# KristinnVikarJ/nbody-simulation

Measured on AMD Instinct MI355X. Metric: pair-interactions/sec + ms/step at N=1M direct O(N^2) (force + integration step), higher is better.
Workload: dtype f32; 1 GPU; direct O(N^2) f32, N=1048576 bodies, seeded 2-D Plummer sphere, masses 1, dt=0.1, clamp=0.001 (BASELINE.json configs[2]); n_bodies=1048576, targets_per_gpu=1048576, n_ranks=1, entry=one process per GPU (sharding.py over nbody_direct_{prep,run}_dev), exchange=none, arith=AUTO (FAST kernel; EXACT on hazardous positions)

## Files before the change

### nbody-simulation_amd/csrc/direct_mutual.hip

```cpp
#include <hip/hip_runtime.h>
#include <stdint.h>

#include "direct_kernels.h"
#include "mutual_schedule.h"

namespace nbody {

namespace {

typedef float v2f __attribute__((ext_vector_type(2)));

constexpr int kWaves = 8;

constexpr int kSlice = kMutualSlice;
constexpr int kSliceCouples = kSlice / 2;
constexpr int kChunks = kSliceCouples / 64;
constexpr float kMarker = 1e30f;

__device__ __forceinline__ bool gate_open(const DirectArgs& a) { return a.run_state < 0 || a.flags[kFlagState] == a.run_state; }

__device__ __forceinline__ float4 couple_or_marker(const float4* c, int64_t k, int64_t n_couples) {
  return k < n_couples ? c[k] : make_float4(kMarker, kMarker, kMarker, kMarker);
}

#define NB_PX(K, H, D) "v_pk_add_f32 v[" D "], v[184:185], %[tx" #K "] op_sel:[0," #H "] op_sel_hi:[1," #H "] neg_lo:[0,1] neg_hi:[0,1]\n\t"
#define NB_PY(K, H, D) "v_pk_add_f32 v[" D "], v[186:187], %[ty" #K "] op_sel:[0," #H "] op_sel_hi:[1," #H "] neg_lo:[0,1] neg_hi:[0,1]\n\t"
#define NB_SQ(DX, DY, Q) "v_pk_mul_f32 v[" Q "], v[" DX "], v[" DX "]\n\tv_pk_fma_f32 v[" Q "], v[" DY "], v[" DY "], v[" Q "]\n\t"
#define NB_AD(XL, XH, YL, YH, SL, SH) "v_add_f32_e64 v" SL ", |v" XL "|, |v" YL "|\n\tv_add_f32_e64 v" SH ", |v" XH "|, |v" YH "|\n\t"
#define NB_DN(S, Q) "v_pk_fma_f32 v[" S "], v[" S "], v[" Q "], %[b]\n\t"
#define NB_RC(SL, SH) "v_rcp_f32_e32 v" SL ", v" SL "\n\tv_rcp_f32_e32 v" SH ", v" SH "\n\t"
#define NB_AC(T, DX, DY, S)                                                                                                          \
  "v_pk_fma_f32 %[ax" #T "], v[" DX "], v[" S "], %[ax" #T "]\n\t"                                                                    \
  "v_pk_fma_f32 v[188:189], v[" DX "], v[" S "], v[188:189] neg_lo:[1,0,0] neg_hi:[1,0,0]\n\t"                                                  \
  "v_pk_fma_f32 %[ay" #T "], v[" DY "], v[" S "], %[ay" #T "]\n\t"                                                                    \
  "v_pk_fma_f32 v[190:191], v[" DY "], v[" S "], v[190:191] neg_lo:[1,0,0] neg_hi:[1,0,0]\n\t"
#define NB_HALF(K0, K1, K2, K3, T0, T1, T2, T3, T4, T5, T6, T7)                                                                    \
  NB_PX(K0, 0, "192:193") NB_PX(K0, 1, "200:201") NB_PX(K1, 0, "208:209") NB_PX(K1, 1, "216:217")                                   \
  NB_PX(K2, 0, "224:225") NB_PX(K2, 1, "232:233") NB_PX(K3, 0, "240:241") NB_PX(K3, 1, "248:249")                                   \
  NB_PY(K0, 0, "194:195") NB_PY(K0, 1, "202:203") NB_PY(K1, 0, "210:211") NB_PY(K1, 1, "218:219")                                   \
  NB_PY(K2, 0, "226:227") NB_PY(K2, 1, "234:235") NB_PY(K3, 0, "242:243") NB_PY(K3, 1, "250:251")                                   \
  NB_SQ("192:193", "194:195", "196:197") NB_SQ("200:201", "202:203", "204:205") NB_SQ("208:209", "210:211", "212:213")             \
  NB_SQ("216:217", "218:219", "220:221") NB_SQ("224:225", "226:227", "228:229") NB_SQ("232:233", "234:235", "236:237")             \
  NB_SQ("240:241", "242:243", "244:245") NB_SQ("248:249", "250:251", "252:253")                                                    \
  "s_setprio 0\n\t"                                                                                                                \
  NB_AD("192", "193", "194", "195", "198", "199") NB_AD("200", "201", "202", "203", "206", "207")                                  \
  NB_AD("208", "209", "210", "211", "214", "215") NB_AD("216", "217", "218", "219", "222", "223")                                  \
  NB_AD("224", "225", "226", "227", "230", "231") NB_AD("232", "233", "234", "235", "238", "239")                                  \
  NB_AD("240", "241", "242", "243", "246", "247") NB_AD("248", "249", "250", "251", "254", "255")                                  \
  "s_setprio 1\n\t"                                                                                                                \
  NB_DN("198:199", "196:197") NB_DN("206:207", "204:205") NB_DN("214:215", "212:213") NB_DN("222:223", "220:221")                 \
  NB_DN("230:231", "228:229") NB_DN("238:239", "236:237") NB_DN("246:247", "244:245") NB_DN("254:255", "252:253")                 \
  NB_RC("198", "199")                                                                                                              \
  NB_RC("206", "207") NB_AC(T0, "192:193", "194:195", "198:199")                                                                   \
  NB_RC("214", "215") NB_AC(T1, "200:201", "202:203", "206:207")                                                                   \
  NB_RC("222", "223") NB_AC(T2, "208:209", "210:211", "214:215")                                                                   \
  NB_RC("230", "231") NB_AC(T3, "216:217", "218:219", "222:223")                                                                   \
  NB_RC("238", "239") NB_AC(T4, "224:225", "226:227", "230:231")                                                                   \
  NB_RC("246", "247") NB_AC(T5, "232:233", "234:235", "238:239")                                                                   \
  NB_RC("254", "255") NB_AC(T6, "240:241", "242:243", "246:247")                                                                   \
  NB_AC(T7, "248:249", "250:251", "254:255")
#define NB_ROT(R) "v_mov_b32_dpp " R ", " R " wave_ror:1 row_mask:0xf bank_mask:0xf\n\t"

__device__ __forceinline__ void mutual_steps(const v2f* tx, const v2f* ty, v2f* ax, v2f* ay, float4& rc, float4& sacc, int steps,
                                             unsigned long long bias2) {
  asm volatile("v_mov_b32 v184, %[r0]\n\tv_mov_b32 v185, %[r1]\n\tv_mov_b32 v186, %[r2]\n\tv_mov_b32 v187, %[r3]\n\t"
               "v_mov_b32 v188, %[o0]\n\tv_mov_b32 v189, %[o1]\n\tv_mov_b32 v190, %[o2]\n\tv_mov_b32 v191, %[o3]\n\t"
               "s_mov_b32 s88, %[n]\n"
               ".Lnb_mutual_%=:\n\t"
               NB_HALF(0, 1, 2, 3, 0, 1, 2, 3, 4, 5, 6, 7) NB_HALF(4, 5, 6, 7, 8, 9, 10, 11, 12, 13, 14, 15)
               NB_ROT("v184") NB_ROT("v185") NB_ROT("v186") NB_ROT("v187") NB_ROT("v188") NB_ROT("v189") NB_ROT("v190") NB_ROT("v191")
               "s_sub_u32 s88, s88, 1\n\t"
               "s_cmp_lg_u32 s88, 0\n\t"
               "s_cbranch_scc1 .Lnb_mutual_%=\n\t"
               "v_mov_b32 %[o0], v188\n\tv_mov_b32 %[o1], v189\n\tv_mov_b32 %[o2], v190\n\tv_mov_b32 %[o3], v191\n\t"
               "v_mov_b32 %[r0], v184\n\tv_mov_b32 %[r1], v185\n\tv_mov_b32 %[r2], v186\n\tv_mov_b32 %[r3], v187\n\t"
               : [ax0] "+v"(ax[0]), [ax1] "+v"(ax[1]), [ax2] "+v"(ax[2]), [ax3] "+v"(ax[3]), [ax4] "+v"(ax[4]), [ax5] "+v"(ax[5]),
                 [ax6] "+v"(ax[6]), [ax7] "+v"(ax[7]), [ax8] "+v"(ax[8]), [ax9] "+v"(ax[9]), [ax10] "+v"(ax[10]), [ax11] "+v"(ax[11]),
                 [ax12] "+v"(ax[12]), [ax13] "+v"(ax[13]), [ax14] "+v"(ax[14]), [ax15] "+v"(ax[15]),
                 [ay0] "+v"(ay[0]), [ay1] "+v"(ay[1]), [ay2] "+v"(ay[2]), [ay3] "+v"(ay[3]), [ay4] "+v"(ay[4]), [ay5] "+v"(ay[5]),
                 [ay6] "+v"(ay[6]), [ay7] "+v"(ay[7]), [ay8] "+v"(ay[8]), [ay9] "+v"(ay[9]), [ay10] "+v"(ay[10]), [ay11] "+v"(ay[11]),
                 [ay12] "+v"(ay[12]), [ay13] "+v"(ay[13]), [ay14] "+v"(ay[14]), [ay15] "+v"(ay[15]),
                 [o0] "+v"(sacc.x), [o1] "+v"(sacc.y), [o2] "+v"(sacc.z), [o3] "+v"(sacc.w),
                 [r0] "+v"(rc.x), [r1] "+v"(rc.y), [r2] "+v"(rc.z), [r3] "+v"(rc.w)
               : [tx0] "v"(tx[0]), [tx1] "v"(tx[1]), [tx2] "v"(tx[2]), [tx3] "v"(tx[3]), [tx4] "v"(tx[4]), [tx5] "v"(tx[5]),
                 [tx6] "v"(tx[6]), [tx7] "v"(tx[7]), [ty0] "v"(ty[0]), [ty1] "v"(ty[1]), [ty2] "v"(ty[2]), [ty3] "v"(ty[3]),
                 [ty4] "v"(ty[4]), [ty5] "v"(ty[5]), [ty6] "v"(ty[6]), [ty7] "v"(ty[7]), [b] "s"(bias2), [n] "s"(steps)
               : "v184", "v185", "v186", "v187", "v188", "v189", "v190", "v191",
                 "v192", "v193", "v194", "v195", "v196", "v197", "v198", "v199", "v200", "v201", "v202", "v203", "v204", "v205",
                 "v206", "v207", "v208", "v209", "v210", "v211", "v212", "v213", "v214", "v215", "v216", "v217", "v218", "v219",
                 "v220", "v221", "v222", "v223", "v224", "v225", "v226", "v227", "v228", "v229", "v230", "v231", "v232", "v233",
                 "v234", "v235", "v236", "v237", "v238", "v239", "v240", "v241", "v242", "v243", "v244", "v245", "v246", "v247",
                 "v248", "v249", "v250", "v251", "v252", "v253", "v254", "v255", "s88", "scc");
}
#undef NB_PX
#undef NB_PY
#undef NB_SQ
#undef NB_AD
#undef NB_DN
#undef NB_RC
#undef NB_AC
#undef NB_HALF
#undef NB_ROT

__device__ __forceinline__ void load_targets(const float4* couples, int64_t n_couples, int s, int w, int lane, v2f* tx, v2f* ty) {
  const int64_t tc0 = (int64_t)s * kSliceCouples + 512 * w + 8 * lane;
#pragma unroll
  for (int k = 0; k < 8; ++k) {
    const float4 c = couple_or_marker(couples, tc0 + k, n_couples);
    tx[k] = v2f{c.x, c.y};
    ty[k] = v2f{c.z, c.w};
  }
}

__device__ __forceinline__ void zero_acc(v2f* ax, v2f* ay) {
#pragma unroll
  for (int t = 0; t < 16; ++t) ax[t] = ay[t] = v2f{0.f, 0.f};
}

__device__ __forceinline__ void add_chunk(const v2f* ax, const v2f* ay, float* tot_x, float* tot_y) {
#pragma unroll
  for (int t = 0; t < 16; ++t) {
    tot_x[t] += ax[t].x + ax[t].y;
    tot_y[t] += ay[t].x + ay[t].y;
  }
}

constexpr unsigned long long kBias2 = 0x1280000012800000ull;

__device__ __forceinline__ void off_item(const float4* couples, int64_t n_couples, int s, int b, int w, int lane, float4 (*red)[kWaves][64],
                                         float2* tpart, float2* spart_f2) {
  v2f tx[8], ty[8];
  load_targets(couples, n_couples, s, w, lane, tx, ty);
  float tot_x[16], tot_y[16];
#pragma unroll
  for (int t = 0; t < 16; ++t) tot_x[t] = tot_y[t] = 0.f;
  float* spart = reinterpret_cast<float*>(spart_f2);
  for (int c = 0; c < kChunks; ++c) {
    float4 rc = couple_or_marker(couples, (int64_t)b * kSliceCouples + 64 * c + lane, n_couples);
    v2f ax[16], ay[16];
    zero_acc(ax, ay);
    float4 sacc = make_float4(0.f, 0.f, 0.f, 0.f);
    mutual_steps(tx, ty, ax, ay, rc, sacc, 64, kBias2);
    add_chunk(ax, ay, tot_x, tot_y);
    red[c & 1][w][lane] = sacc;
    __syncthreads();
    if (threadIdx.x < 256) {
      const int q = threadIdx.x >> 2, comp = threadIdx.x & 3;
      float r = 0.f;
#pragma unroll
      for (int v = 0; v < kWaves; ++v) r += reinterpret_cast<const float*>(&red[c & 1][v][q])[comp];
      spart[(size_t)(128 * c + 2 * q + (comp & 1)) * 2 + (comp >> 1)] = r;
    }
  }
#pragma unroll
  for (int t = 0; t < 16; ++t) tpart[1024 * w + 16 * lane + t] = make_float2(tot_x[t], tot_y[t]);
}

__device__ __forceinline__ void diag_item(const float4* couples, int64_t n_couples, int s, int w, int lane, float4 (*src)[8][64],
                                          float2* out) {
  using namespace mutual_schedule;
  v2f tx[8], ty[8];
  load_targets(couples, n_couples, s, w, lane, tx, ty);
  float tot_x[16], tot_y[16];
#pragma unroll
  for (int t = 0; t < 16; ++t) tot_x[t] = tot_y[t] = 0.f;
  const int64_t c0 = (int64_t)s * kSliceCouples;
  for (int p = 0; p < kDiagPhases; ++p) {
    const int u = diag_block(w, p), r0 = diag_first_step(w, p), n = diag_steps(p);
    for (int j = 0; j < 8; ++j) {
      float4 rc = couple_or_marker(couples, c0 + 512 * u + 8 * ((lane - r0) & 63) + j, n_couples);
      v2f ax[16], ay[16];
      zero_acc(ax, ay);
      float4 sacc = make_float4(0.f, 0.f, 0.f, 0.f);
      int moved;
      if (p == 0) {
        mutual_steps(tx, ty, ax, ay, rc, sacc, 1, kBias2);
        sacc = make_float4(0.f, 0.f, 0.f, 0.f);
        mutual_steps(tx, ty, ax, ay, rc, sacc, n - 2, kBias2);
        const float4 keep = sacc;
        mutual_steps(tx, ty, ax, ay, rc, sacc, 1, kBias2);
        sacc = keep;
        moved = n - 1;
      } else {
        mutual_steps(tx, ty, ax, ay, rc, sacc, n, kBias2);
        moved = n;
      }
      add_chunk(ax, ay, tot_x, tot_y);
      const int shift = (r0 + moved) & 63;
      if (shift) {
        const int from = (lane + shift) & 63;
        sacc = make_float4(__shfl(sacc.x, from), __shfl(sacc.y, from), __shfl(sacc.z, from), __shfl(sacc.w, from));
      }
      float4& d = src[u][j][lane];
      if (p == 0) {
        d = sacc;
      } else {
        const float4 o = d;
        d = make_float4(o.x + sacc.x, o.y + sacc.y, o.z + sacc.z, o.w + sacc.w);
      }
    }
    __syncthreads();
  }
#pragma unroll
  for (int k = 0; k < 8; ++k) {
    const float4 q = src[w][k][lane];
    out[1024 * w + 16 * lane + 2 * k] = make_float2(tot_x[2 * k] + q.x, tot_y[2 * k] + q.z);
    out[1024 * w + 16 * lane + 2 * k + 1] = make_float2(tot_x[2 * k + 1] + q.y, tot_y[2 * k + 1] + q.w);
  }
  __syncthreads();
}

__global__ __launch_bounds__(kWaves * 64) void direct_mutual(const DirectArgs a, MutualArea m, int64_t lo) {
  if (!gate_open(a)) return;
  const int nb = m.n_slices;
  int s, b;
  mutual_schedule::unit_slices(lo + blockIdx.x, nb, s, b);
  const int lane = threadIdx.x & 63;
  const int w = __builtin_amdgcn_readfirstlane((int)(threadIdx.x >> 6));
  const float4* couples = reinterpret_cast<const float4*>(a.src_pos);
  const int64_t n_couples = a.n_src / 2;
  float2* tpart = m.tpart + (size_t)blockIdx.x * kSlice;
  float2* spart = m.spart + (size_t)blockIdx.x * kSlice;
  __shared__ float4 lds[8][8][64];
  __builtin_amdgcn_s_setprio(1);
  if (s < b) {
    off_item(couples, n_couples, s, b, w, lane, reinterpret_cast<float4(*)[kWaves][64]>(&lds[0][0][0]), tpart, spart);
  } else {
    diag_item(couples, n_couples, s, w, lane, lds, tpart);
    if (s + 1 < nb) diag_item(couples, n_couples, s + 1, w, lane, lds, spart);
  }
}

__global__ __launch_bounds__(256) void direct_mutual_near(const DirectArgs a, MutualArea m) {
  if (!gate_open(a)) return;
  const int n_near = a.flags[kFlagNearCount];
  const float4* couples = reinterpret_cast<const float4*>(a.src_pos);
  const int n_couples = a.n_src / 2;
  const int per = (n_couples + kMutualNearSplit - 1) / kMutualNearSplit;
  const int q0 = blockIdx.x * per, q1 = q0 + per < n_couples ? q0 + per : n_couples;
  __shared__ float2 red[256];
  for (int k = blockIdx.y; k < n_near; k += gridDim.y) {
    const float2 p = a.pos_all[a.near_list[k]];
    float ax = 0.f, ay = 0.f;
#pragma unroll 4
    for (int q = q0 + (int)threadIdx.x; q < q1; q += 256) {
      const float4 c = couples[q];
#pragma unroll
      for (int h = 0; h < 2; ++h) {
        const float dx = (h ? c.y : c.x) - p.x, dy = (h ? c.w : c.z) - p.y;
        const float sum = __builtin_fabsf(dx) + __builtin_fabsf(dy);
        const float d2 = __builtin_fmaf(dy, dy, dx * dx);
        const float s = __builtin_amdgcn_rcpf(__builtin_fmaf(sum, d2, 8.0779356694631609e-28f));
        ax = __builtin_fmaf(dx, s, ax);
        ay = __builtin_fmaf(dy, s, ay);
      }
    }
    red[threadIdx.x] = make_float2(ax, ay);
    __syncthreads();
    for (int w = 128; w > 0; w >>= 1) {
      if ((int)threadIdx.x < w) {
        red[threadIdx.x].x += red[threadIdx.x + w].x;
        red[threadIdx.x].y += red[threadIdx.x + w].y;
      }
      __syncthreads();
    }
    if (threadIdx.x == 0) m.near_part[(size_t)k * kMutualNearSplit + blockIdx.x] = red[0];
    __syncthreads();
  }
}

__global__ __launch_bounds__(256) void direct_mutual_reduce(const DirectArgs a, MutualArea m, int64_t lo, int64_t hi, int first, int last) {
  using mutual_schedule::item_of;
  if (!gate_open(a)) return;
  const int i = blockIdx.x * 256 + threadIdx.x;
  if (i >= a.n_tgt) return;
  const int nb = m.n_slices;
  const int s = i / kSlice, l = i % kSlice;
  int r0 = 0, r1 = s;
  while (r0 < r1) {
    const int mid = (r0 + r1) >> 1;
    if (item_of(mid, s, nb) < lo) r0 = mid + 1; else r1 = mid;
  }
  int re = s;
  r1 = r0;
  while (r1 < re) {
    const int mid = (r1 + re) >> 1;
    if (item_of(mid, s, nb) < hi) r1 = mid + 1; else re = mid;
  }
  const int64_t b0 = s + 1 < nb ? item_of(s, s + 1, nb) : 0, b1 = s + 1 < nb ? item_of(s, nb - 1, nb) + 1 : 0;
  const int64_t w0 = b0 > lo ? b0 : lo, w1 = b1 < hi ? b1 : hi;
  const int64_t d = mutual_schedule::diag_unit(s, nb);
  const bool has_d = d >= lo && d < hi;
  if (r0 == r1 && w0 >= w1 && !has_d && !first && !last) return;
  float2 acc = first ? make_float2(0.f, 0.f) : a.partial[i];
#pragma unroll 8
  for (int r = r0; r < r1; ++r) {
    const float2 p = m.spart[(size_t)(item_of(r, s, nb) - lo) * kSlice + l];
    acc.x += p.x;
    acc.y += p.y;
  }
#pragma unroll 8
  for (int64_t it = w0; it < w1; ++it) {
    const float2 p = m.tpart[(size_t)(it - lo) * kSlice + l];
    acc.x += p.x;
    acc.y += p.y;
  }
  if (has_d) {
    const float2 p = ((s & 1) ? m.spart : m.tpart)[(size_t)(d - lo) * kSlice + l];
    acc.x += p.x;
    acc.y += p.y;
  }
  if (last) {
    if (m.is_near[i]) {
      const float2* np = m.near_part + (size_t)m.near_scan[i] * kMutualNearSplit;
      acc = np[0];
      for (int g = 1; g < kMutualNearSplit; ++g) {
        acc.x += np[g].x;
        acc.y += np[g].y;
      }
    }
    acc = make_float2(acc.x * a.uniform_mass, acc.y * a.uniform_mass);
  }
  a.partial[i] = acc;
}

}

int mutual_slices(int64_t n_slots) { return (int)((n_slots + kSlice - 1) / kSlice); }

size_t mutual_area_bytes(int64_t n_src) {
  return 2 * (size_t)kMutualStripItems * kSlice * sizeof(float2) + ((size_t)n_src / 64 + 2) * kMutualNearSplit * sizeof(float2);
}

MutualArea mutual_area(void* base, int64_t n_src, const uint32_t* is_near, const uint32_t* near_scan) {
  MutualArea m{};
  m.n_slices = mutual_slices(far_padded(n_src));
  float2* p = (float2*)base;
  m.tpart = p;
  p += (size_t)kMutualStripItems * kSlice;
  m.spart = p;
  p += (size_t)kMutualStripItems * kSlice;
  m.near_part = p;
  m.is_near = is_near;
  m.near_scan = near_scan;
  return m;
}

hipError_t launch_direct_mutual(hipStream_t s, const DirectArgs& a, const MutualArea& m) {
  if (a.n_tgt <= 0) return hipSuccess;
  if (!a.src_couples || a.tgt_begin != 0 || a.n_src < a.n_tgt || m.n_slices != mutual_slices(a.n_src)) return hipErrorInvalidValue;
  int dev = 0, cus = 0;
  hipError_t e = hipGetDevice(&dev);
  if (e == hipSuccess) e = hipDeviceGetAttribute(&cus, hipDeviceAttributeMultiprocessorCount, dev);
  if (e != hipSuccess) return e;
  if (cus <= 0) return hipErrorInvalidValue;
  const int64_t units = mutual_schedule::units(m.n_slices);
  const int64_t strip = mutual_schedule::strip_units(cus, kMutualStripItems);
  const dim3 rgrid((unsigned)((a.n_tgt + 255) / 256));
  hipLaunchKernelGGL(direct_mutual_near, dim3(kMutualNearSplit, kMutualNearRows), dim3(256), 0, s, a, m);
  for (int64_t lo = 0; lo < units; lo += strip) {
    const int64_t hi = lo + strip < units ? lo + strip : units;
    hipLaunchKernelGGL(direct_mutual, dim3((unsigned)(hi - lo)), dim3(kWaves * 64), 0, s, a, m, lo);
    hipLaunchKernelGGL(direct_mutual_reduce, rgrid, dim3(256), 0, s, a, m, lo, hi, lo == 0 ? 1 : 0, hi == units ? 1 : 0);
  }
  return hipGetLastError();
}

}
```

### nbody-simulation_amd/csrc/mutual_schedule.h

```cpp
#pragma once
#include <stdint.h>

#if defined(__HIPCC__)
#define NB_HD __host__ __device__
#else
#define NB_HD
#endif

namespace nbody {
namespace mutual_schedule {

NB_HD inline int64_t off_items(int nb) { return (int64_t)nb * (nb - 1) / 2; }
NB_HD inline int64_t item_of(int s, int b, int nb) { return (int64_t)s * nb - (int64_t)s * (s + 1) / 2 + (b - s - 1); }
NB_HD inline int64_t units(int nb) { return off_items(nb) + (nb + 1) / 2; }
NB_HD inline void unit_slices(int64_t unit, int nb, int& s, int& b) {
  const int64_t n_off = off_items(nb);
  if (unit < n_off) {
    s = 0;
    int64_t first = 0;
    while (first + (nb - 1 - s) <= unit) first += nb - 1 - s++;
    b = s + 1 + (int)(unit - first);
  } else {
    s = b = 2 * (int)(unit - n_off);
  }
}
NB_HD inline int64_t diag_unit(int s, int nb) { return off_items(nb) + s / 2; }

NB_HD inline int strip_units(int cus, int capacity) { return cus >= capacity ? capacity : capacity / cus * cus; }

constexpr int kDiagPhases = 5;
NB_HD inline int diag_block(int w, int p) { return (w + p) & 7; }
NB_HD inline int diag_first_step(int w, int p) { return p == 4 && w >= 4 ? 1 : 0; }
NB_HD inline int diag_steps(int p) { return p == 0 ? 33 : p == 4 ? 32 : 64; }
NB_HD inline bool diag_one_sided(int p, int i) { return p == 0 && (i == 0 || i == 32); }

}
}

#undef NB_HD
```

Baseline: 10070 billion pair-interactions/s.

## Prefetch next off-diagonal chunk in asm and keep chunk accumulators in fixed registers

```diff
diff --git a/nbody-simulation_amd/csrc/direct_mutual.hip b/nbody-simulation_amd/csrc/direct_mutual.hip
--- a/nbody-simulation_amd/csrc/direct_mutual.hip
+++ b/nbody-simulation_amd/csrc/direct_mutual.hip
@@ -14,7 +14,7 @@
 
 constexpr int kSlice = kMutualSlice;
 constexpr int kSliceCouples = kSlice / 2;
-constexpr int kChunks = kSliceCouples / 64;
+constexpr int kChunks = kSliceCouples / mutual_schedule::kChunkCouples;
 constexpr float kMarker = 1e30f;
 
 __device__ __forceinline__ bool gate_open(const DirectArgs& a) { return a.run_state < 0 || a.flags[kFlagState] == a.run_state; }
@@ -29,12 +29,48 @@
 #define NB_AD(XL, XH, YL, YH, SL, SH) "v_add_f32_e64 v" SL ", |v" XL "|, |v" YL "|\n\tv_add_f32_e64 v" SH ", |v" XH "|, |v" YH "|\n\t"
 #define NB_DN(S, Q) "v_pk_fma_f32 v[" S "], v[" S "], v[" Q "], %[b]\n\t"
 #define NB_RC(SL, SH) "v_rcp_f32_e32 v" SL ", v" SL "\n\tv_rcp_f32_e32 v" SH ", v" SH "\n\t"
-#define NB_AC(T, DX, DY, S)                                                                                                          \
-  "v_pk_fma_f32 %[ax" #T "], v[" DX "], v[" S "], %[ax" #T "]\n\t"                                                                    \
-  "v_pk_fma_f32 v[188:189], v[" DX "], v[" S "], v[188:189] neg_lo:[1,0,0] neg_hi:[1,0,0]\n\t"                                                  \
-  "v_pk_fma_f32 %[ay" #T "], v[" DY "], v[" S "], %[ay" #T "]\n\t"                                                                    \
+#define NB_OPX(T) "%[ax" #T "]"
+#define NB_OPY(T) "%[ay" #T "]"
+#define NB_FXX(T) NB_FXX_##T
+#define NB_FXY(T) NB_FXY_##T
+#define NB_FXX_0 "v[120:121]"
+#define NB_FXY_0 "v[122:123]"
+#define NB_FXX_1 "v[124:125]"
+#define NB_FXY_1 "v[126:127]"
+#define NB_FXX_2 "v[128:129]"
+#define NB_FXY_2 "v[130:131]"
+#define NB_FXX_3 "v[132:133]"
+#define NB_FXY_3 "v[134:135]"
+#define NB_FXX_4 "v[136:137]"
+#define NB_FXY_4 "v[138:139]"
+#define NB_FXX_5 "v[140:141]"
+#define NB_FXY_5 "v[142:143]"
+#define NB_FXX_6 "v[144:145]"
+#define NB_FXY_6 "v[146:147]"
+#define NB_FXX_7 "v[148:149]"
+#define NB_FXY_7 "v[150:151]"
+#define NB_FXX_8 "v[152:153]"
+#define NB_FXY_8 "v[154:155]"
+#define NB_FXX_9 "v[156:157]"
+#define NB_FXY_9 "v[158:159]"
+#define NB_FXX_10 "v[160:161]"
+#define NB_FXY_10 "v[162:163]"
+#define NB_FXX_11 "v[164:165]"
+#define NB_FXY_11 "v[166:167]"
+#define NB_FXX_12 "v[168:169]"
+#define NB_FXY_12 "v[170:171]"
+#define NB_FXX_13 "v[172:173]"
+#define NB_FXY_13 "v[174:175]"
+#define NB_FXX_14 "v[176:177]"
+#define NB_FXY_14 "v[178:179]"
+#define NB_FXX_15 "v[180:181]"
+#define NB_FXY_15 "v[182:183]"
+#define NB_AC(A, T, DX, DY, S)                                                                                                       \
+  "v_pk_fma_f32 " A##X(T) ", v[" DX "], v[" S "], " A##X(T) "\n\t"                                                                    \
+  "v_pk_fma_f32 v[188:189], v[" DX "], v[" S "], v[188:189] neg_lo:[1,0,0] neg_hi:[1,0,0]\n\t"                                      \
+  "v_pk_fma_f32 " A##Y(T) ", v[" DY "], v[" S "], " A##Y(T) "\n\t"                                                                    \
   "v_pk_fma_f32 v[190:191], v[" DY "], v[" S "], v[190:191] neg_lo:[1,0,0] neg_hi:[1,0,0]\n\t"
-#define NB_HALF(K0, K1, K2, K3, T0, T1, T2, T3, T4, T5, T6, T7)                                                                    \
+#define NB_HALF(A, K0, K1, K2, K3, T0, T1, T2, T3, T4, T5, T6, T7)                                                                    \
   NB_PX(K0, 0, "192:193") NB_PX(K0, 1, "200:201") NB_PX(K1, 0, "208:209") NB_PX(K1, 1, "216:217")                                   \
   NB_PX(K2, 0, "224:225") NB_PX(K2, 1, "232:233") NB_PX(K3, 0, "240:241") NB_PX(K3, 1, "248:249")                                   \
   NB_PY(K0, 0, "194:195") NB_PY(K0, 1, "202:203") NB_PY(K1, 0, "210:211") NB_PY(K1, 1, "218:219")                                   \
@@ -51,14 +87,14 @@
   NB_DN("198:199", "196:197") NB_DN("206:207", "204:205") NB_DN("214:215", "212:213") NB_DN("222:223", "220:221")                 \
   NB_DN("230:231", "228:229") NB_DN("238:239", "236:237") NB_DN("246:247", "244:245") NB_DN("254:255", "252:253")                 \
   NB_RC("198", "199")                                                                                                              \
-  NB_RC("206", "207") NB_AC(T0, "192:193", "194:195", "198:199")                                                                   \
-  NB_RC("214", "215") NB_AC(T1, "200:201", "202:203", "206:207")                                                                   \
-  NB_RC("222", "223") NB_AC(T2, "208:209", "210:211", "214:215")                                                                   \
-  NB_RC("230", "231") NB_AC(T3, "216:217", "218:219", "222:223")                                                                   \
-  NB_RC("238", "239") NB_AC(T4, "224:225", "226:227", "230:231")                                                                   \
-  NB_RC("246", "247") NB_AC(T5, "232:233", "234:235", "238:239")                                                                   \
-  NB_RC("254", "255") NB_AC(T6, "240:241", "242:243", "246:247")                                                                   \
-  NB_AC(T7, "248:249", "250:251", "254:255")
+  NB_RC("206", "207") NB_AC(A, T0, "192:193", "194:195", "198:199")                                                                   \
+  NB_RC("214", "215") NB_AC(A, T1, "200:201", "202:203", "206:207")                                                                   \
+  NB_RC("222", "223") NB_AC(A, T2, "208:209", "210:211", "214:215")                                                                   \
+  NB_RC("230", "231") NB_AC(A, T3, "216:217", "218:219", "222:223")                                                                   \
+  NB_RC("238", "239") NB_AC(A, T4, "224:225", "226:227", "230:231")                                                                   \
+  NB_RC("246", "247") NB_AC(A, T5, "232:233", "234:235", "238:239")                                                                   \
+  NB_RC("254", "255") NB_AC(A, T6, "240:241", "242:243", "246:247")                                                                   \
+  NB_AC(A, T7, "248:249", "250:251", "254:255")
 #define NB_ROT(R) "v_mov_b32_dpp " R ", " R " wave_ror:1 row_mask:0xf bank_mask:0xf\n\t"
 
 __device__ __forceinline__ void mutual_steps(const v2f* tx, const v2f* ty, v2f* ax, v2f* ay, float4& rc, float4& sacc, int steps,
@@ -67,7 +103,7 @@
                "v_mov_b32 v188, %[o0]\n\tv_mov_b32 v189, %[o1]\n\tv_mov_b32 v190, %[o2]\n\tv_mov_b32 v191, %[o3]\n\t"
                "s_mov_b32 s88, %[n]\n"
                ".Lnb_mutual_%=:\n\t"
-               NB_HALF(0, 1, 2, 3, 0, 1, 2, 3, 4, 5, 6, 7) NB_HALF(4, 5, 6, 7, 8, 9, 10, 11, 12, 13, 14, 15)
+               NB_HALF(NB_OP, 0, 1, 2, 3, 0, 1, 2, 3, 4, 5, 6, 7) NB_HALF(NB_OP, 4, 5, 6, 7, 8, 9, 10, 11, 12, 13, 14, 15)
                NB_ROT("v184") NB_ROT("v185") NB_ROT("v186") NB_ROT("v187") NB_ROT("v188") NB_ROT("v189") NB_ROT("v190") NB_ROT("v191")
                "s_sub_u32 s88, s88, 1\n\t"
                "s_cmp_lg_u32 s88, 0\n\t"
@@ -92,6 +128,69 @@
                  "v234", "v235", "v236", "v237", "v238", "v239", "v240", "v241", "v242", "v243", "v244", "v245", "v246", "v247",
                  "v248", "v249", "v250", "v251", "v252", "v253", "v254", "v255", "s88", "scc");
 }
+
+#define NB_Z2(D) "v_mov_b64 v[" D "], 0\n\t"
+#define NB_FOLD(T, XL, XH, YL, YH, SL, SH)                                                                                          \
+  "v_add_f32_e32 v" SL ", v" XL ", v" XH "\n\tv_add_f32_e32 v" SH ", v" YL ", v" YH "\n\t"                                             \
+  "v_pk_add_f32 %[tot" #T "], %[tot" #T "], v[" SL ":" SH "]\n\t"
+__device__ __forceinline__ void off_chunk(const v2f* tx, const v2f* ty, v2f* tot, float4& rc, float4& sacc, const float4* base,
+                                          unsigned voff, unsigned long long lanes, unsigned long long bias2) {
+  asm volatile("v_mov_b32 v188, 0\n\tv_mov_b32 v189, 0\n\tv_mov_b32 v190, 0\n\tv_mov_b32 v191, 0\n\t"
+               "v_mov_b32 v116, 0x7149f2ca\n\tv_mov_b32 v117, 0x7149f2ca\n\tv_mov_b32 v118, 0x7149f2ca\n\tv_mov_b32 v119, 0x7149f2ca\n\t"
+               "s_mov_b64 s[90:91], exec\n\t"
+               "s_mov_b64 exec, %[lanes]\n\t"
+               "global_load_dwordx4 v[116:119], %[voff], %[base]\n\t"
+               "s_mov_b64 exec, s[90:91]\n\t"
+               NB_Z2("120:121") NB_Z2("122:123") NB_Z2("124:125") NB_Z2("126:127")
+               NB_Z2("128:129") NB_Z2("130:131") NB_Z2("132:133") NB_Z2("134:135")
+               NB_Z2("136:137") NB_Z2("138:139") NB_Z2("140:141") NB_Z2("142:143")
+               NB_Z2("144:145") NB_Z2("146:147") NB_Z2("148:149") NB_Z2("150:151")
+               NB_Z2("152:153") NB_Z2("154:155") NB_Z2("156:157") NB_Z2("158:159")
+               NB_Z2("160:161") NB_Z2("162:163") NB_Z2("164:165") NB_Z2("166:167")
+               NB_Z2("168:169") NB_Z2("170:171") NB_Z2("172:173") NB_Z2("174:175")
+               NB_Z2("176:177") NB_Z2("178:179") NB_Z2("180:181") NB_Z2("182:183")
+               "s_mov_b32 s88, 64\n"
+               ".Lnb_chunk_%=:\n\t"
+               NB_HALF(NB_FX, 0, 1, 2, 3, 0, 1, 2, 3, 4, 5, 6, 7) NB_HALF(NB_FX, 4, 5, 6, 7, 8, 9, 10, 11, 12, 13, 14, 15)
+               NB_ROT("v184") NB_ROT("v185") NB_ROT("v186") NB_ROT("v187") NB_ROT("v188") NB_ROT("v189") NB_ROT("v190") NB_ROT("v191")
+               "s_sub_u32 s88, s88, 1\n\t"
+               "s_cmp_lg_u32 s88, 0\n\t"
+               "s_cbranch_scc1 .Lnb_chunk_%=\n\t"
+               NB_FOLD(0, "120", "121", "122", "123", "192", "193") NB_FOLD(1, "124", "125", "126", "127", "194", "195")
+               NB_FOLD(2, "128", "129", "130", "131", "196", "197") NB_FOLD(3, "132", "133", "134", "135", "198", "199")
+               NB_FOLD(4, "136", "137", "138", "139", "200", "201") NB_FOLD(5, "140", "141", "142", "143", "202", "203")
+               NB_FOLD(6, "144", "145", "146", "147", "204", "205") NB_FOLD(7, "148", "149", "150", "151", "206", "207")
+               NB_FOLD(8, "152", "153", "154", "155", "208", "209") NB_FOLD(9, "156", "157", "158", "159", "210", "211")
+               NB_FOLD(10, "160", "161", "162", "163", "212", "213") NB_FOLD(11, "164", "165", "166", "167", "214", "215")
+               NB_FOLD(12, "168", "169", "170", "171", "216", "217") NB_FOLD(13, "172", "173", "174", "175", "218", "219")
+               NB_FOLD(14, "176", "177", "178", "179", "220", "221") NB_FOLD(15, "180", "181", "182", "183", "222", "223")
+               "s_waitcnt vmcnt(0)\n\t"
+               "v_mov_b32 v184, v116\n\tv_mov_b32 v185, v117\n\tv_mov_b32 v186, v118\n\tv_mov_b32 v187, v119\n\t"
+               : [tot0] "+v"(tot[0]), [tot1] "+v"(tot[1]), [tot2] "+v"(tot[2]), [tot3] "+v"(tot[3]), [tot4] "+v"(tot[4]),
+                 [tot5] "+v"(tot[5]), [tot6] "+v"(tot[6]), [tot7] "+v"(tot[7]), [tot8] "+v"(tot[8]), [tot9] "+v"(tot[9]),
+                 [tot10] "+v"(tot[10]), [tot11] "+v"(tot[11]), [tot12] "+v"(tot[12]), [tot13] "+v"(tot[13]), [tot14] "+v"(tot[14]),
+                 [tot15] "+v"(tot[15]),
+                 "+{v184}"(rc.x), "+{v185}"(rc.y), "+{v186}"(rc.z), "+{v187}"(rc.w),
+                 "=&{v188}"(sacc.x), "=&{v189}"(sacc.y), "=&{v190}"(sacc.z), "=&{v191}"(sacc.w)
+               : [tx0] "v"(tx[0]), [tx1] "v"(tx[1]), [tx2] "v"(tx[2]), [tx3] "v"(tx[3]), [tx4] "v"(tx[4]), [tx5] "v"(tx[5]),
+                 [tx6] "v"(tx[6]), [tx7] "v"(tx[7]), [ty0] "v"(ty[0]), [ty1] "v"(ty[1]), [ty2] "v"(ty[2]), [ty3] "v"(ty[3]),
+                 [ty4] "v"(ty[4]), [ty5] "v"(ty[5]), [ty6] "v"(ty[6]), [ty7] "v"(ty[7]), [b] "s"(bias2), [base] "s"(base),
+                 [voff] "v"(voff), [lanes] "s"(lanes)
+               :
+                 "v116", "v117", "v118", "v119", "v120", "v121", "v122", "v123", "v124", "v125", "v126", "v127", "v128", "v129",
+                 "v130", "v131", "v132", "v133", "v134", "v135", "v136", "v137", "v138", "v139", "v140", "v141", "v142", "v143",
+                 "v144", "v145", "v146", "v147", "v148", "v149", "v150", "v151", "v152", "v153", "v154", "v155", "v156", "v157",
+                 "v158", "v159", "v160", "v161", "v162", "v163", "v164", "v165", "v166", "v167", "v168", "v169", "v170", "v171",
+                 "v172", "v173", "v174", "v175", "v176", "v177", "v178", "v179", "v180", "v181", "v182", "v183",
+                 "v192", "v193", "v194", "v195", "v196", "v197", "v198", "v199", "v200", "v201", "v202", "v203", "v204", "v205",
+                 "v206", "v207", "v208", "v209", "v210", "v211", "v212", "v213", "v214", "v215", "v216", "v217", "v218", "v219",
+                 "v220", "v221", "v222", "v223", "v224", "v225", "v226", "v227", "v228", "v229", "v230", "v231", "v232", "v233",
+                 "v234", "v235", "v236", "v237", "v238", "v239", "v240", "v241", "v242", "v243", "v244", "v245", "v246", "v247",
+                 "v248", "v249", "v250", "v251", "v252", "v253", "v254", "v255",
+                 "s88", "s90", "s91", "scc");
+}
+#undef NB_Z2
+#undef NB_FOLD
 #undef NB_PX
 #undef NB_PY
 #undef NB_SQ
@@ -99,6 +198,10 @@
 #undef NB_DN
 #undef NB_RC
 #undef NB_AC
+#undef NB_OPX
+#undef NB_OPY
+#undef NB_FXX
+#undef NB_FXY
 #undef NB_HALF
 #undef NB_ROT
 
@@ -127,21 +230,24 @@
 
 constexpr unsigned long long kBias2 = 0x1280000012800000ull;
 
-__device__ __forceinline__ void off_item(const float4* couples, int64_t n_couples, int s, int b, int w, int lane, float4 (*red)[kWaves][64],
+__device__ __forceinline__ void off_item(const float4* couples, int64_t n_couples, int s, int b, int w, float4 (*red)[kWaves][64],
                                          float2* tpart, float2* spart_f2) {
+  using namespace mutual_schedule;
+  const int lane = (int)__builtin_amdgcn_mbcnt_hi(~0u, __builtin_amdgcn_mbcnt_lo(~0u, 0u));
   v2f tx[8], ty[8];
   load_targets(couples, n_couples, s, w, lane, tx, ty);
-  float tot_x[16], tot_y[16];
-#pragma unroll
-  for (int t = 0; t < 16; ++t) tot_x[t] = tot_y[t] = 0.f;
+  v2f tot[16];
+#pragma unroll
+  for (int t = 0; t < 16; ++t) tot[t] = v2f{0.f, 0.f};
   float* spart = reinterpret_cast<float*>(spart_f2);
+  const unsigned voff = (unsigned)lane * (unsigned)sizeof(float4);
+  float4 rc = couple_or_marker(couples, off_chunk_first(b, 0, kSliceCouples) + lane, n_couples);
   for (int c = 0; c < kChunks; ++c) {
-    float4 rc = couple_or_marker(couples, (int64_t)b * kSliceCouples + 64 * c + lane, n_couples);
-    v2f ax[16], ay[16];
-    zero_acc(ax, ay);
-    float4 sacc = make_float4(0.f, 0.f, 0.f, 0.f);
-    mutual_steps(tx, ty, ax, ay, rc, sacc, 64, kBias2);
-    add_chunk(ax, ay, tot_x, tot_y);
+    const int cn = off_prefetched(c, kChunks);
+    const int64_t first = off_chunk_first(b, cn < 0 ? c : cn, kSliceCouples);
+    const unsigned long long lanes = cn < 0 ? 0ull : chunk_lanes(first, n_couples);
+    float4 sacc;
+    off_chunk(tx, ty, tot, rc, sacc, couples + first, voff, lanes, kBias2);
     red[c & 1][w][lane] = sacc;
     __syncthreads();
     if (threadIdx.x < 256) {
@@ -153,7 +259,7 @@
     }
   }
 #pragma unroll
-  for (int t = 0; t < 16; ++t) tpart[1024 * w + 16 * lane + t] = make_float2(tot_x[t], tot_y[t]);
+  for (int t = 0; t < 16; ++t) tpart[1024 * w + 16 * lane + t] = make_float2(tot[t].x, tot[t].y);
 }
 
 __device__ __forceinline__ void diag_item(const float4* couples, int64_t n_couples, int s, int w, int lane, float4 (*src)[8][64],
@@ -224,7 +330,7 @@
   __shared__ float4 lds[8][8][64];
   __builtin_amdgcn_s_setprio(1);
   if (s < b) {
-    off_item(couples, n_couples, s, b, w, lane, reinterpret_cast<float4(*)[kWaves][64]>(&lds[0][0][0]), tpart, spart);
+    off_item(couples, n_couples, s, b, w, reinterpret_cast<float4(*)[kWaves][64]>(&lds[0][0][0]), tpart, spart);
   } else {
     diag_item(couples, n_couples, s, w, lane, lds, tpart);
     if (s + 1 < nb) diag_item(couples, n_couples, s + 1, w, lane, lds, spart);
diff --git a/nbody-simulation_amd/csrc/mutual_schedule.h b/nbody-simulation_amd/csrc/mutual_schedule.h
--- a/nbody-simulation_amd/csrc/mutual_schedule.h
+++ b/nbody-simulation_amd/csrc/mutual_schedule.h
@@ -34,6 +34,14 @@
 NB_HD inline int diag_steps(int p) { return p == 0 ? 33 : p == 4 ? 32 : 64; }
 NB_HD inline bool diag_one_sided(int p, int i) { return p == 0 && (i == 0 || i == 32); }
 
+constexpr int kChunkCouples = 64;
+NB_HD inline int64_t off_chunk_first(int b, int c, int slice_couples) { return (int64_t)b * slice_couples + (int64_t)kChunkCouples * c; }
+NB_HD inline int off_prefetched(int c, int chunks) { return c + 1 < chunks ? c + 1 : -1; }
+NB_HD inline uint64_t chunk_lanes(int64_t first, int64_t n_couples) {
+  const int64_t left = n_couples - first;
+  return left >= kChunkCouples ? ~0ull : left <= 0 ? 0ull : (1ull << left) - 1;
+}
+
 }
 }
 
```

Result: no change. 10110 billion pair-interactions/s (median of 6 runs) (+0.3%).
